# joezie/Personalized-PageRank-Algorithms-on-Neo4j

Hardware: AMD Instinct MI355X
Metric: single-source PPR queries/sec (FORA, alpha=0.15, eps=0.5) (higher is better)
Workload: dtype f64

## Files before the change

### personalized-pagerank-algorithms-on-neo4j_amd/csrc/engine.hpp

```cpp
#pragma once

#include <atomic>
#include <cstdlib>
#include <vector>

#include "common.hpp"

namespace pprhip {

constexpr int kMaxBatch = 8;

struct DevCounters {
  unsigned long long hist[16];
  unsigned long long packed[2];
  double dead[2];
  unsigned long long dead_pops;
  unsigned long long walk_steps;
  unsigned long long walks_total;
  unsigned long long sources_total;
  unsigned long long walk_loads;
  unsigned long long walk_lanes;
  double sum_out;
  unsigned long long mc_plan[3];
  double plan_sum[3];
// ... 164 lines not shown
    if (!last_timed) return;
    last_timed = false;
    hipEvent_t b = next();
    if (b) (void)hipEventRecord(b, stream);
  }
  void add_bytes(int cls, uint64_t bytes) { acc_bytes[cls] += bytes; }
  void reset() {
    used = 0;
    depth = 0;
    last_timed = false;
    recs.clear();
    for (int c = 0; c < 8; ++c) {
      acc_ms[c] = 0.0;
      acc_bytes[c] = 0;
      acc_cnt[c] = 0;
    }
  }
  void resolve(double tot[8], uint64_t bytes[8], uint32_t cnt[8]) {
    fold();
    for (int c = 0; c < 8; ++c) {
      tot[c] += acc_ms[c];
      bytes[c] += acc_bytes[c];
      cnt[c] += acc_cnt[c];
    }
  }
  void destroy() {
    for (hipEvent_t e : ev) (void)hipEventDestroy(e);
    ev.clear();
    reset();
  }
};

struct BatchSync;

constexpr int kBatch = 16;
struct CView {
  double* p;
  uint32_t stride, off;
  __host__ __device__ double& at(uint32_t v) const { return p[(size_t)v * stride + off]; }
};

struct SlotArgs {
  double* res;
  double* reserve;
  uint8_t* flags;
  uint32_t* armed;
  DevCounters* ctr;
  double alpha, rmax, min_rmax;
  int32_t src;
  int32_t active;
  int32_t mode;
  int32_t dead_slot, out_slot;
  int32_t gs_state;
  const double* seed_w;
  const int32_t* seed_id;
  const double* seed_e;
  unsigned int* seed_done;
  uint32_t seed_n_live, seed_n_all;
};

constexpr uint32_t kMailWords = 4112;
struct HostMail {
  unsigned long long seq;
  unsigned long long pad[7];
  unsigned long long words[kMailWords];
};

struct ClearList {
  void* p[6];
  unsigned long long bytes[6];
  int n;
};

struct WalkPlanRec {
  unsigned long long woff;
  double inc;
  unsigned long long ext;
  int32_t node, orig;
};

}

namespace pprhip {
namespace detail {
struct FetchPipe;
}

struct GraphData {
  int device = 0;
  int n_cus = 256;
  uint32_t n = 0;
  uint64_t m = 0;
  uint32_t *out_rp = nullptr, *in_rp = nullptr;
  unsigned long long* out_ext = nullptr;
  int32_t *out_ci = nullptr, *in_ci = nullptr;
  uint4* walk_rec = nullptr;
  std::vector<uint32_t> h_out_rp, h_in_rp;
  bool relabeled = false;
  int32_t *new2old = nullptr, *old2new = nullptr;
  std::vector<int32_t> h_new2old, h_old2new;
  uint8_t* start_flags = nullptr;
  uint32_t* chunk_starts = nullptr;
  uint32_t n_chunks = 0;
  int32_t* nz_rows = nullptr;
  uint32_t n_nz = 0;
  std::vector<int32_t> h_nz_rows;
// ... 240 lines not shown
```

### personalized-pagerank-algorithms-on-neo4j_amd/csrc/fora.cpp

```cpp
#include <algorithm>
#include <atomic>
#include <chrono>
#include <cmath>
#include <condition_variable>
#include <cstdio>
#include <cstring>
#include <functional>
#include <memory>
#include <mutex>
#include <new>
#include <thread>

#include "engine_internal.hpp"

using namespace pprhip;
using namespace pprhip::detail;

namespace pprhip {

struct TopkSchedule {
  double eps = 0, min_delta = 0, m = 0, lg = 0, min_rmax = 0;
  TopkSchedule() = default;
  TopkSchedule(double eps_half, const pprhip_fora_conf_t* conf)
      : eps(eps_half), min_delta(conf->min_delta), m((double)conf->m), lg(std::log(2.0 / conf->pfail)),
// ... 646 lines not shown
  PPRHIP_TRY(check_conf(conf, "pprhip_fora_topk", true));
  PPRHIP_TRY(check_graph(g, "pprhip_fora_topk"));
  PPRHIP_TRY(check_node(g, src, "pprhip_fora_topk"));
  if (!fora_topk_args_ok(conf, eps, cap, ids_out, vals_out, "pprhip_fora_topk")) return PPRHIP_ERR_INVALID;
  ForaRun r;
  PPRHIP_TRY(topk_begin(r, g, g->gr->h_old2new[src], eps, conf, seed, ids_out, vals_out, cap));
  return fora_topk_drive(r, n_out, reserve_out, stats);
}

int pprhip_fora_topk_seeds(pprhip_graph_t* g, const int32_t* seeds, const double* weights, int n_seeds, double eps,
                           const pprhip_fora_conf_t* conf, uint64_t seed, int32_t* ids_out, double* vals_out, int cap,
                           int* n_out, double* reserve_out, pprhip_stats_t* stats) {
  static const char* fn = "pprhip_fora_topk_seeds";
  PPRHIP_TRY(check_positive(eps, fn, "eps"));
  PPRHIP_TRY(check_conf(conf, fn, true));
  PPRHIP_TRY(check_graph(g, fn));
  if (!fora_topk_args_ok(conf, eps, cap, ids_out, vals_out, fn)) return PPRHIP_ERR_INVALID;
  SeedTable plan;
  PPRHIP_TRY(seed_plan(g, seeds, weights, n_seeds, conf->alpha, fn, plan));
  ForaRun r;
  PPRHIP_TRY(topk_begin_seeds(r, g, plan, eps, conf, seed, ids_out, vals_out, cap));
  const int rc = fora_topk_drive(r, n_out, reserve_out, stats);
  g->topk_active = false;
  return rc;
}

namespace {

struct SweepTicket {
  bool active[kBatch] = {false};
  int ws[kBatch] = {0};
  int n_active = 0;
  bool backward = false;
  uint64_t rows = 0;
  unsigned long long seq = 0;
};

int launch_sweep(pprhip_graph* P, ForaRun* runs, const bool* active, int n_active, SweepTicket* T, const int* ws = nullptr) {
  BatchState* bs = P->batch;
  const GraphData* D = P->gr;
  T->n_active = n_active;
  int n_seeded = 0;
  for (int s = 0; s < kBatch; ++s) {
    T->ws[s] = (ws && active[s]) ? ws[s] : s;
    pprhip_graph* S = bs->slots[T->ws[s]];
    SlotArgs& sa = bs->h_slot_args[s];
    T->active[s] = active[s];
    sa.res = S->residue;
    sa.reserve = S->reserve;
    sa.flags = S->flags;
    sa.armed = S->armed;
    sa.ctr = S->ctr;
    sa.active = active[s] ? 1 : 0;
    const SeedTable* sd = (active[s] && S->seed_on) ? S->seeds : nullptr;
    sa.seed_w = sd ? sd->w_node : nullptr;
    sa.seed_id = sd ? sd->id : nullptr;
    sa.seed_e = sd ? sd->w : nullptr;
    sa.seed_done = sd ? sd->done : nullptr;
    sa.seed_n_live = sd ? sd->n_live : 0u;
    sa.seed_n_all = sd ? sd->n_live + sd->n_dead : 0u;
    n_seeded += sd ? 1 : 0;
    if (!active[s]) continue;
    const ForaRun& r = runs[T->ws[s]];
    sa.alpha = r.a.alpha;
    sa.rmax = r.a.rmax;
    sa.min_rmax = r.a.min_rmax;
    sa.src = r.a.src;
    sa.mode = r.a.mode;
    sa.dead_slot = r.L.dslot;
    sa.out_slot = r.L.pslot ^ 1;
    sa.gs_state = r.L.gs_state;
    if (S->stream != P->stream && !S->c8_via_parent) {
      PPRHIP_CHECK_HIP(hipEventRecord(S->ev[3], S->stream));
      PPRHIP_CHECK_HIP(hipStreamWaitEvent(P->stream, S->ev[3], 0));
    }
  }
  bool backward = false;
  for (int s = 0; s < kBatch; ++s)
    if (active[s] && runs[T->ws[s]].a.mode == kBackward) backward = true;
  T->backward = backward;
  const uint64_t rows = backward ? (uint64_t)D->n_nz_o + D->n_z_o : (uint64_t)D->n_nz + D->n_zin;
  T->rows = rows;
  const uint64_t sweep_bytes =
      4ull * D->m + (uint64_t)n_active * (8ull * D->m + 36ull * rows + 4ull) + (uint64_t)n_seeded * 8ull * rows;
  if ((int)backward != bs->acc8_dir) {
    PPRHIP_CHECK_HIP(hipMemsetAsync(bs->acc8, 0, sizeof(double) * ((size_t)D->n + 1) * kBatch, P->stream));
    bs->acc8_dir = (int)backward;
  }
  int n_gs = 1;
  const GsBlock* gs_blocks = backward ? nullptr : gs_blocks_of(bs->slots[0], &n_gs);
#ifdef PPRHIP_TEST_HOOKS
  {
    static const bool on = hook_env("PPRHIP_COUNT_LIVE") != nullptr;
    static unsigned long long* d_cnt = nullptr;
    static unsigned long long sweeps = 0;
    if (on && !backward) {
      if (!d_cnt) {
        PPRHIP_CHECK_HIP(hipMalloc((void**)&d_cnt, 16));
        PPRHIP_CHECK_HIP(hipMemset(d_cnt, 0, 16));
      }
      PPRHIP_TRY(launch_count_live_lines(P, d_cnt));
      if (++sweeps % 200 == 0) {
        unsigned long long h[2];
        PPRHIP_CHECK_HIP(hipMemcpy(h, d_cnt, 16, hipMemcpyDeviceToHost));
        fprintf(stderr, "[pprhip live lines] %llu sweeps: gathers of live lines %.3f of m, live lines %.3f of the sources, busy columns now %d\n",
                sweeps, (double)h[0] / (double)sweeps / (double)D->m, (double)h[1] / (double)sweeps / (double)D->n_src_live, n_active);
      }
    }
  }
#endif
  P->ktimer.begin(PPRHIP_KERNEL_DENSE_PULL_BATCH, sweep_bytes);
  PPRHIP_TRY(launch_dense_level_b8(P, backward, gs_blocks, n_gs));
  P->ktimer.end();
  bs->c8cur ^= 1;
  return fetch_begin(P, bs->sweep_out, sizeof(unsigned long long) * kBatch, &T->seq);
}

bool sweep_arrived(const pprhip_graph* P, const SweepTicket& T) {
  return T.seq != 0 && P->mail && __atomic_load_n(&P->mail->seq, __ATOMIC_ACQUIRE) == T.seq;
}

int collect_sweep(pprhip_graph* P, ForaRun* runs, const SweepTicket& T) {
  PPRHIP_TRY(fetch_end(P, T.seq, P->batch->sweep_out, P->batch->h_sweep_out, sizeof(unsigned long long) * kBatch));
  for (int s = 0; s < kBatch; ++s)
    if (T.active[s]) {
      ForaRun& r = runs[T.ws[s]];
      const unsigned long long pk = P->batch->h_sweep_out[s];
      finish_dense(r.L, r.st, 8ull * P->gr->m + 36ull * T.rows + 4ull + 4ull * P->gr->m / (uint64_t)T.n_active,
                   batch_sweep_min_bytes(P, T.backward, T.n_active) / (uint64_t)T.n_active, (uint32_t)(pk >> kPackShift),
                   pk & kPackMask);
    }
  return PPRHIP_OK;
}

int run_sweep(pprhip_graph* P, ForaRun* runs, const bool* active, int n_active) {
  SweepTicket T;
  PPRHIP_TRY(launch_sweep(P, runs, active, n_active, &T));
// ... 1327 lines not shown
```

### personalized-pagerank-algorithms-on-neo4j_amd/csrc/kernels_push.hip

```cpp
#include <algorithm>
#include <cstdlib>

#include "device_utils.hpp"
#include "engine.hpp"

namespace pprhip {

constexpr int kPushTile = 2048;
constexpr int kStageCap = 512;
constexpr int kCombSlots = 2048;
constexpr int kCombProbes = 4;
constexpr int kCombMinEdges = 262144;

__device__ __forceinline__ bool level_runs(unsigned long long pk, int level, unsigned long long dense_thresh) {
  if (level == 0) return true;
  const unsigned long long nf = pk >> kPackShift, ef = pk & kPackMask;
  if (nf == 0) return false;
  return (nf + ef) < dense_thresh;
}

__device__ __forceinline__ int dense_state(const int* state_in, int state0) { return state_in ? *state_in : state0; }

template <int MODE>
__device__ __forceinline__ void sparse_prepare_body(const int32_t* __restrict__ F, const uint32_t* __restrict__ out_rp,
                                                    double* __restrict__ res, double* __restrict__ reserve,
                                                    double* __restrict__ cF, CView c_dense, DevCounters* ctr, int level,
                                                    int dead_slot, unsigned long long pk0, unsigned long long pk,
                                                    const PushArgs& a, uint32_t bid, uint32_t nblk) {
  __shared__ double s_red[4];
  __shared__ unsigned long long s_red2[4];
  if (level == 0 && pk0 != ~0ull && bid == 0 && threadIdx.x == 0) {
    for (int i = 1; i <= kMaxBatch; ++i) ctr->hist[i] = 0ull;
    ctr->hist[kMaxBatch + 2] = 0ull;
  }
  const uint32_t nf = (uint32_t)(pk >> kPackShift);
  double dead = 0.0;
  unsigned long long ndead = 0;
  for (uint32_t i = bid * blockDim.x + threadIdx.x; i < nf; i += nblk * blockDim.x) {
    const int32_t v = F[i];
    const double rc = res[v];
    res[v] = 0.0;
    reserve[v] = reserve[v] + rc * a.alpha;
    double c;
    if (MODE == kBackward) {
      c = (1.0 - a.alpha) * rc;
    } else {
      const uint32_t d = out_rp[v + 1] - out_rp[v];
      if (d == 0) {
        c = 0.0;
        dead += rc * (1.0 - a.alpha);
        ndead++;
      } else {
        c = ((1.0 - a.alpha) * rc) / (double)d;
// ... 810 lines not shown
    if (MODE == kBackward) {
      if (acc > 0.0) {
        const double old = res[u];
        const double nw = old + acc / (double)d;
        if (!(old > a.rmax) && nw > a.rmax) {
          reserve[u] = reserve[u] + nw * a.alpha;
          if (old != 0.0) res[u] = 0.0;
          cn = (1.0 - a.alpha) * nw;
          pack = (1ull << kPackShift) | (unsigned long long)(in_rp[u + 1] - in_rp[u]);
        } else {
          res[u] = nw;
        }
      }
    } else if (acc > 0.0) {
      const double old = res[u];
      const double nw = old + acc;
      bool crossing = (MODE == kPower) ? true : (!active_fwd(old, d, a.rmax) && active_fwd(nw, d, a.rmax));
      if (MODE == kFwdTopk) {
        if (a.rmax < a.min_rmax && active_fwd(old, d, a.rmax)) crossing = take_armed(armed, u);
        if (active_fwd(nw, d, a.min_rmax)) flags[u] = 1;
      }
      if (crossing) {
        reserve[u] = reserve[u] + nw * a.alpha;
        if (old != 0.0) res[u] = 0.0;
        if (d == 0) {
          dead_next = nw * (1.0 - a.alpha);
          ndead = 1;
        } else {
          cn = ((1.0 - a.alpha) * nw) / (double)d;
        }
        pack = (1ull << kPackShift) | (unsigned long long)d;
      } else {
        res[u] = nw;
      }
    }
    c_next[u] = cn;
    if (!last_block) {
      if (state == kGsEntry) c_cur[u] = c_cur[u] + cn;
      else if (state == kGsInPlace) c_cur[u] = cn;
      else if (state == kGsFlush) c_cur[u] = 0.0;
    }
  }
  const double ds = block_sum_f64(dead_next, s_red);
  const unsigned long long ps = block_sum_u64(pack, s_red2);
  const unsigned long long nd = block_sum_u64(ndead, s_red2);
  if (tid == 0) {
    blk_pack[blockIdx.x] = ps;
    blk_dead[blockIdx.x] = ds;
    blk_ndead[blockIdx.x] = (uint32_t)nd;
  }
}

constexpr int kApplyRows = 64;
constexpr int kApplyGroups = 2;
constexpr int kApplyThreads = 512;
constexpr int kSlotsPerWave = kBatch / (kApplyThreads / 64);

__global__ __launch_bounds__(kApplyThreads) void k_dense_apply_batch(const int32_t* __restrict__ nz_rows, uint32_t n_nz,
                                                            const int32_t* __restrict__ zin_rows, uint32_t n_zin,
                                                            double* __restrict__ acc8,
                                                            const uint32_t* __restrict__ out_rp,
                                                            const uint32_t* __restrict__ in_rp_bwd,
                                                            double* __restrict__ c8_cur, double* __restrict__ c8_next,
                                                            uint32_t tile_lo, uint32_t tile_hi, uint32_t gs_mask,
                                                            uint32_t entry_mask,
                                                            const SlotArgs* __restrict__ slots,
                                                            const unsigned long long* __restrict__ cross_bits,
                                                            unsigned long long* __restrict__ prep_bits,
                                                            unsigned long long* __restrict__ blk_pack8,
                                                            double* __restrict__ blk_dead8,
                                                            uint32_t* __restrict__ blk_ndead8, uint32_t part_base,
                                                            uint32_t part_stride) {
  __shared__ double tile[kApplyGroups][kApplyRows][kBatch + 1];
  __shared__ double tile_p[kApplyGroups][kApplyRows][kBatch + 1];
  __shared__ int32_t s_u[kApplyGroups][kApplyRows];
  __shared__ uint32_t s_d[kApplyGroups][kApplyRows];
  __shared__ uint32_t s_din[kApplyGroups][kApplyRows];
  const int tid = threadIdx.x, lane = tid & 63;
  const int w = __builtin_amdgcn_readfirstlane(tid >> 6);
  const uint32_t n_rows = n_nz + n_zin;
  const uint32_t n_tiles = (n_rows + kApplyRows - 1) / kApplyRows;
  SlotArgs a[kSlotsPerWave];
#pragma unroll
  for (int i = 0; i < kSlotsPerWave; ++i) a[i] = slots[w * kSlotsPerWave + i];
  double dead_next[kSlotsPerWave];
  unsigned long long pack[kSlotsPerWave];
  uint32_t ndead[kSlotsPerWave];
#pragma unroll
  for (int i = 0; i < kSlotsPerWave; ++i) {
    dead_next[i] = 0.0;
    pack[i] = 0;
    ndead[i] = 0;
  }
  for (uint32_t tl0 = tile_lo + blockIdx.x * kApplyGroups; tl0 < tile_hi; tl0 += gridDim.x * kApplyGroups) {
#pragma unroll
    for (int g = 0; g < kApplyGroups; ++g) {
      const uint32_t tl = tl0 + g;
      const bool in = tl < tile_hi;
      const uint32_t row0 = tl * kApplyRows;
      const unsigned long long cw = in ? cross_bits[tl] : 0ull;
#pragma unroll
      for (int i = 0; i < kApplyRows * kBatch / kApplyThreads; ++i) {
        const uint32_t idx = (uint32_t)i * (uint32_t)kApplyThreads + tid;
        const uint32_t r = idx / kBatch, s = idx % kBatch;
        const uint32_t j = row0 + r;
        double v = 0.0;
        if (in && j < n_nz) {
          const size_t t = (size_t)j * kBatch + s;
          v = __builtin_nontemporal_load(&acc8[t]);
          if (v != 0.0 && ((cw >> r) & 1ull)) acc8[t] = 0.0;
        }
// ... 88 lines not shown
          }
          if (crossing) {
            a[i].reserve[u[g]] = rsvv[g][i] + nw * a[i].alpha;
            if (oldv[g][i] != 0.0) a[i].res[u[g]] = 0.0;
            if (d[g] == 0) {
              dead_next[i] += nw * (1.0 - a[i].alpha);
              ndead[i]++;
            } else {
              cn = ((1.0 - a[i].alpha) * nw) / (double)d[g];
            }
            pack[i] += (1ull << kPackShift) | (unsigned long long)d[g];
          } else {
            a[i].res[u[g]] = nw;
          }
        }
        tile[g][lane][s] = cn;
        if (gs_mask >> s & 1u) {
          const int gst = a[i].gs_state;
          tile_p[g][lane][s] = gst == kGsEntry ? tile_p[g][lane][s] + cn : (gst == kGsInPlace ? cn : 0.0);
        }
        const unsigned long long bits = __ballot(cn > 0.0);
        if (lane == 0 && a[i].active && tl0 + g < tile_hi) prep_bits[(size_t)s * n_tiles + tl0 + g] = bits;
      }
    }
    __syncthreads();
#pragma unroll
    for (int g = 0; g < kApplyGroups; ++g) {
#pragma unroll
      for (int i = 0; i < kApplyRows * kBatch / kApplyThreads; ++i) {
        const uint32_t idx = (uint32_t)i * (uint32_t)kApplyThreads + tid;
        const uint32_t r = idx / kBatch, s = idx % kBatch;
        const int32_t ur = s_u[g][r];
        if (ur >= 0) {
          c8_next[(size_t)ur * kBatch + s] = tile[g][r][s];
          if (gs_mask >> s & 1u) c8_cur[(size_t)ur * kBatch + s] = tile_p[g][r][s];
        }
      }
    }
    __syncthreads();
  }
#pragma unroll
  for (int i = 0; i < kSlotsPerWave; ++i) {
    const double ds = wave_sum_f64(dead_next[i]);
    const unsigned long long ps = wave_sum_u64(pack[i]);
    const unsigned long long nd = wave_sum_u64((unsigned long long)ndead[i]);
    if (lane == 0) {
      const size_t o = (size_t)(w * kSlotsPerWave + i) * part_stride + part_base + blockIdx.x;
      blk_pack8[o] = ps;
      blk_dead8[o] = ds;
      blk_ndead8[o] = (uint32_t)nd;
    }
  }
}

__global__ __launch_bounds__(1024) void k_dense_reduce_batch(const unsigned long long* __restrict__ blk_pack8,
                                                           const double* __restrict__ blk_dead8,
                                                           const uint32_t* __restrict__ blk_ndead8, uint32_t n_blocks,
                                                           uint32_t part_stride,
                                                           const SlotArgs* __restrict__ slots,
                                                           unsigned long long* __restrict__ sweep_out) {
  __shared__ double s_red[16];
  __shared__ unsigned long long s_red2[16];
  const SlotArgs a = slots[blockIdx.x];
  if (!a.active) return;
  unsigned long long pack = 0, ndead = 0;
  double dead = 0.0;
  for (uint32_t i = threadIdx.x; i < n_blocks; i += blockDim.x) {
    pack += blk_pack8[(size_t)blockIdx.x * part_stride + i];
    dead += blk_dead8[(size_t)blockIdx.x * part_stride + i];
    ndead += blk_ndead8[(size_t)blockIdx.x * part_stride + i];
  }
  const unsigned long long ps = block_sum_u64(pack, s_red2);
  const unsigned long long nd = block_sum_u64(ndead, s_red2);
  const double ds = block_sum_f64(dead, s_red);
  if (threadIdx.x == 0) {
    a.ctr->packed[a.out_slot] = ps;
    sweep_out[blockIdx.x] = ps;
    if (nd) {
      a.ctr->dead[a.dead_slot ^ 1] = a.ctr->dead[a.dead_slot ^ 1] + ds;
      a.ctr->dead_pops += nd;
    }
  }
}

__global__ __launch_bounds__(1024) void k_dense_reduce(const unsigned long long* __restrict__ blk_pack,
                                                        const double* __restrict__ blk_dead,
                                                        const uint32_t* __restrict__ blk_ndead, uint32_t n_blocks,
                                                        DevCounters* ctr, int out_slot, int dead_slot_next,
                                                        const int* state_in, int state0, unsigned long long* hist_out,
                                                        int* state_out, unsigned long long dense_thresh,
                                                        unsigned long long gs_thresh, uint32_t* queues) {
  __shared__ double s_red[16];
  __shared__ unsigned long long s_red2[16];
  if (queues && threadIdx.x < kPanelQueues) queues[threadIdx.x] = 0u;
  const int state = dense_state(state_in, state0);
  if (state == kGsNone) {
    if (threadIdx.x == 0 && state_out) *state_out = kGsNone;
    return;
  }
  unsigned long long pack = 0, ndead = 0;
  double dead = 0.0;
  for (uint32_t i = threadIdx.x; i < n_blocks; i += blockDim.x) {
    pack += blk_pack[i];
    if (blk_dead) {
      dead += blk_dead[i];
      ndead += blk_ndead[i];
    }
  }
  const unsigned long long ps = block_sum_u64(pack, s_red2);
  const unsigned long long nd = block_sum_u64(ndead, s_red2);
  const double ds = block_sum_f64(dead, s_red);
  if (threadIdx.x == 0) {
    ctr->packed[out_slot] = ps;
    if (hist_out) *hist_out = ps;
    if (state_out) *state_out = gs_next_state(state, ps >> kPackShift, ps & kPackMask, dense_thresh, gs_thresh);
    if (nd) {
      ctr->dead[dead_slot_next] = ctr->dead[dead_slot_next] + ds;
      ctr->dead_pops += nd;
    }
  }
}

template <int KIND>
__device__ __forceinline__ bool seed_pred(uint32_t v, const double* __restrict__ res, uint32_t d,
                                          const uint8_t* __restrict__ flags, const PushArgs& a) {
  if (KIND == 1 && !flags[v]) return false;
  return active_fwd(res[v], d, a.rmax);
}

__device__ __forceinline__ void unpark(uint32_t v, const double* __restrict__ res, uint32_t d,
                                       uint8_t* __restrict__ flags, const PushArgs& a) {
  if (!flags[v]) return;
  const double r = res[v];
  if (active_fwd(r, d, a.rmax) || !active_fwd(r, d, a.min_rmax)) flags[v] = 0;
}

template <int KIND>
// ... 537 lines not shown
  const uint32_t c_hi = (uint32_t)((B.e_hi + kChunkEdges - 1) / kChunkEdges);
  const uint32_t want = (c_hi - c_lo + 15) / 16;
  const unsigned long long* flags64 = reinterpret_cast<const unsigned long long*>(start_flags);
  if (n_hot) {
    const uint32_t grid = std::min<uint32_t>(want, (uint32_t)g->gr->n_cus);
    k_dense_edges_b<true, G><<<dim3(grid), dim3(1024), sizeof(double) * n_hot * G, g->stream>>>(
        ci, flags64, chunk_starts, c_hi, (unsigned long long)g->gr->m, cB, accB, n_hot, c_lo, B.e_lo, B.e_hi, g->gr->n);
  } else {
    const uint32_t grid = std::min<uint32_t>(want, (uint32_t)g->gr->n_cus * 2u);
    k_dense_edges_b<false, G><<<dim3(grid), dim3(1024), 0, g->stream>>>(
        ci, flags64, chunk_starts, c_hi, (unsigned long long)g->gr->m, cB, accB, 0u, c_lo, B.e_lo, B.e_hi, g->gr->n);
  }
  PPRHIP_CHECK_HIP(hipGetLastError());
  return PPRHIP_OK;
}

#ifdef PPRHIP_TEST_HOOKS
__global__ __launch_bounds__(256) void k_count_live_lines(const double* __restrict__ c8, const uint32_t* __restrict__ out_rp,
                                                          uint32_t n, unsigned long long* out) {
  __shared__ unsigned long long s_red[4];
  const uint32_t v = blockIdx.x * 256u + threadIdx.x;
  unsigned long long d = 0, c = 0;
  if (v < n) {
    bool live = false;
    for (int s = 0; s < kBatch; ++s) live |= c8[(size_t)v * kBatch + s] != 0.0;
    if (live) {
      d = out_rp[v + 1] - out_rp[v];
      c = 1;
    }
  }
  const unsigned long long ds = block_sum_u64(d, s_red), cs = block_sum_u64(c, s_red);
  if (threadIdx.x == 0 && (ds | cs)) {
    atomicAdd(&out[0], ds);
    atomicAdd(&out[1], cs);
  }
}
int launch_count_live_lines(pprhip_graph* P, unsigned long long* d_out) {
  const BatchState* bs = P->batch;
  k_count_live_lines<<<dim3((P->gr->n + 255) / 256), dim3(256), 0, P->stream>>>(bs->c8[bs->c8cur], P->gr->out_rp, P->gr->n,
                                                                              d_out);
  PPRHIP_CHECK_HIP(hipGetLastError());
  return PPRHIP_OK;
}
#endif

#ifdef PPRHIP_TEST_HOOKS
int launch_sweep_edges_only(pprhip_graph* P, const GsBlock& B) {
  const GraphData* D = P->gr;
  const BatchState* bs = P->batch;
  return launch_dense_edges_bG<kBatch>(P, D->in_ci, D->start_flags, D->chunk_starts, bs->c8[bs->c8cur], bs->acc8, B);
}
#endif

int launch_dense_level_b8(pprhip_graph* P, bool backward, const GsBlock* gs_blocks, int n_gs_blocks) {
  const GraphData* D = P->gr;
  const BatchState* bs = P->batch;
  PPRHIP_CHECK_HIP(hipMemcpyAsync(bs->d_slot_args, bs->h_slot_args, sizeof(SlotArgs) * kBatch, hipMemcpyHostToDevice,
                                  P->stream));
  const int32_t* ci = backward ? D->out_ci : D->in_ci;
  const uint8_t* flags = backward ? D->start_flags_o : D->start_flags;
  const uint32_t* cstarts = backward ? D->chunk_starts_o : D->chunk_starts;
  const int32_t* nz = backward ? D->nz_rows_o : D->nz_rows;
  const int32_t* zr = backward ? D->z_rows_o : D->zin_rows;
  const uint32_t n_nz = backward ? D->n_nz_o : D->n_nz, n_z = backward ? D->n_z_o : D->n_zin;
  const unsigned long long* cross = backward ? D->cross_bits_o : D->cross_bits;
  uint32_t gs_mask = 0, entry_mask = 0;
  for (int s = 0; s < kBatch; ++s)
    if (bs->h_slot_args[s].active) {
      const int st = bs->h_slot_args[s].gs_state;
      if (st == kGsEntry || st == kGsInPlace || st == kGsFlush) gs_mask |= 1u << s;
      if (st == kGsEntry) entry_mask |= 1u << s;
    }
  const uint32_t n_rows = n_nz + n_z;
  const uint32_t n_tiles = (n_rows + kApplyRows - 1) / kApplyRows;
  const GsBlock whole{0u, n_nz, 0ull, (unsigned long long)D->m};
  const bool cut = gs_mask && gs_blocks && n_gs_blocks > 1 && !backward;
  const GsBlock* blocks = cut ? gs_blocks : &whole;
  const int nb = cut ? n_gs_blocks : 1;
  uint32_t part_base = 0;
  for (int b = 0; b < nb; ++b) {
    const GsBlock& B = blocks[b];
    PPRHIP_TRY(launch_dense_edges_bG<kBatch>(P, ci, flags, cstarts, bs->c8[bs->c8cur], bs->acc8, B));
    const uint32_t t_lo = B.j_lo / kApplyRows;
    const uint32_t t_hi = (b == nb - 1) ? n_tiles : B.j_hi / kApplyRows;
    if (t_hi <= t_lo) continue;
    const uint32_t quota = kApplyBlocks8 / (uint32_t)nb;
    const uint32_t grid = std::max(1u, std::min((t_hi - t_lo + kApplyGroups - 1) / kApplyGroups, quota));
    k_dense_apply_batch<<<dim3(grid), dim3(kApplyThreads), 0, P->stream>>>(
          nz, n_nz, zr, n_z, bs->acc8, D->out_rp, backward ? D->in_rp : nullptr, bs->c8[bs->c8cur], bs->c8[bs->c8cur ^ 1], t_lo,
          t_hi, b == nb - 1 ? 0u : gs_mask, b == nb - 1 ? 0u : entry_mask, bs->d_slot_args, cross, bs->prep_bits,
          bs->blk_pack8, bs->blk_dead8, bs->blk_ndead8, part_base, kApplyBlocks8);
    PPRHIP_CHECK_HIP(hipGetLastError());
    part_base += grid;
  }
  uint32_t seed_dead_max = 0;
  bool seeded = false;
  for (int s = 0; s < kBatch; ++s) {
    const SlotArgs& sa = bs->h_slot_args[s];
    if (sa.active && sa.seed_w && !backward) {
      seeded = true;
      seed_dead_max = std::max(seed_dead_max, sa.seed_n_all - sa.seed_n_live);
    }
  }
  if (seeded) {
    k_seed_land_dense_batch<<<dim3(grid_for(seed_dead_max, 256, 1024), kBatch), dim3(256), 0, P->stream>>>(
        bs->d_slot_args);
    PPRHIP_CHECK_HIP(hipGetLastError());
  }
  k_dense_reduce_batch<<<dim3(kBatch), dim3(1024), 0, P->stream>>>(bs->blk_pack8, bs->blk_dead8, bs->blk_ndead8, part_base,
                                                                   kApplyBlocks8, bs->d_slot_args, bs->sweep_out);
  PPRHIP_CHECK_HIP(hipGetLastError());
  return PPRHIP_OK;
}

int launch_compact_prepared(pprhip_graph* g, int cbuf, int out_fbuf, unsigned long long* d_counter, bool backward) {
  const uint32_t grid = grid_for(g->gr->n, 1024, 1024);
  if (g->parent) {
    const GraphData* D = g->gr;
    const uint32_t n_rows = backward ? D->n_nz_o + D->n_z_o : D->n_nz + D->n_zin;
    const uint32_t n_tiles = (n_rows + kApplyRows - 1) / kApplyRows;
    k_compact_bits<<<dim3(grid), dim3(256), 0, g->stream>>>(
        n_rows, backward ? D->n_nz_o : D->n_nz, g->parent->batch->prep_bits + (size_t)g->slot_index * n_tiles,
        backward ? D->nz_rows_o : D->nz_rows, backward ? D->z_rows_o : D->zin_rows, cview(g, cbuf),
        backward ? D->in_rp : D->out_rp, g->F[out_fbuf], g->eoff[out_fbuf], g->cF, d_counter);
  } else {
    k_compact_prepared<<<dim3(grid), dim3(256), 0, g->stream>>>(act_n(g), cview(g, cbuf), false,
                                                                backward ? g->gr->in_rp : g->gr->out_rp, g->F[out_fbuf],
                                                                g->eoff[out_fbuf], g->cF, d_counter);
  }
  PPRHIP_CHECK_HIP(hipGetLastError());
  return PPRHIP_OK;
}

static int reduce_partials(pprhip_graph* g, uint32_t n_blocks, int out_slot, int dead_slot, bool with_dead) {
  k_dense_reduce<<<dim3(1), dim3(1024), 0, g->stream>>>(g->blk_pack, with_dead ? g->blk_dead : nullptr, g->blk_ndead,
                                                        n_blocks, g->ctr, out_slot, dead_slot, nullptr, kGsJacobi, nullptr,
                                                        nullptr, 0ull, ~0ull, nullptr);
  PPRHIP_CHECK_HIP(hipGetLastError());
  return PPRHIP_OK;
}

// ... 127 lines not shown
```

Measured before the change: 346.7.

## Skip residue loads for rows known zero via previous-sweep prep bits

Adds a new dense apply kernel that uses per-tile prep bits written by the previous sweep to skip loading residue (and often reserve) for rows known to hold zero residue, when the slot is in whole-forward mode with a prior dense run. The kernel also double-buffers the shared tile so the write-out of the previous tile overlaps the next tile's work, and it records ballot bits of nonzero outputs for the next sweep. The old kernel is kept behind an environment switch, and the bandwidth estimate is reduced accordingly. The risk is correctness if the prep bits go stale, plus extra shared memory and register pressure.

```diff
diff --git a/personalized-pagerank-algorithms-on-neo4j_amd/csrc/engine.hpp b/personalized-pagerank-algorithms-on-neo4j_amd/csrc/engine.hpp
--- a/personalized-pagerank-algorithms-on-neo4j_amd/csrc/engine.hpp
+++ b/personalized-pagerank-algorithms-on-neo4j_amd/csrc/engine.hpp
@@ -240,6 +240,7 @@
   int32_t mode;
   int32_t dead_slot, out_slot;
   int32_t gs_state;
+  int32_t prep_ok;
   const double* seed_w;
   const int32_t* seed_id;
   const double* seed_e;
diff --git a/personalized-pagerank-algorithms-on-neo4j_amd/csrc/fora.cpp b/personalized-pagerank-algorithms-on-neo4j_amd/csrc/fora.cpp
--- a/personalized-pagerank-algorithms-on-neo4j_amd/csrc/fora.cpp
+++ b/personalized-pagerank-algorithms-on-neo4j_amd/csrc/fora.cpp
@@ -722,6 +722,7 @@
     sa.armed = S->armed;
     sa.ctr = S->ctr;
     sa.active = active[s] ? 1 : 0;
+    sa.prep_ok = 0;
     const SeedTable* sd = (active[s] && S->seed_on) ? S->seeds : nullptr;
     sa.seed_w = sd ? sd->w_node : nullptr;
     sa.seed_id = sd ? sd->id : nullptr;
@@ -740,6 +741,7 @@
     sa.dead_slot = r.L.dslot;
     sa.out_slot = r.L.pslot ^ 1;
     sa.gs_state = r.L.gs_state;
+    sa.prep_ok = (r.a.mode == kFwdWhole && r.L.dense_run > 0) ? 1 : 0;
     if (S->stream != P->stream && !S->c8_via_parent) {
       PPRHIP_CHECK_HIP(hipEventRecord(S->ev[3], S->stream));
       PPRHIP_CHECK_HIP(hipStreamWaitEvent(P->stream, S->ev[3], 0));
@@ -751,8 +753,10 @@
   T->backward = backward;
   const uint64_t rows = backward ? (uint64_t)D->n_nz_o + D->n_z_o : (uint64_t)D->n_nz + D->n_zin;
   T->rows = rows;
-  const uint64_t sweep_bytes =
-      4ull * D->m + (uint64_t)n_active * (8ull * D->m + 36ull * rows + 4ull) + (uint64_t)n_seeded * 8ull * rows;
+  int n_prep = 0;
+  for (int s = 0; s < kBatch; ++s) n_prep += active[s] && bs->h_slot_args[s].prep_ok ? 1 : 0;
+  const uint64_t sweep_bytes = 4ull * D->m + (uint64_t)n_active * (8ull * D->m + 36ull * rows + 4ull) +
+                               (uint64_t)n_seeded * 8ull * rows - (uint64_t)n_prep * 8ull * rows;
   if ((int)backward != bs->acc8_dir) {
     PPRHIP_CHECK_HIP(hipMemsetAsync(bs->acc8, 0, sizeof(double) * ((size_t)D->n + 1) * kBatch, P->stream));
     bs->acc8_dir = (int)backward;
diff --git a/personalized-pagerank-algorithms-on-neo4j_amd/csrc/kernels_push.hip b/personalized-pagerank-algorithms-on-neo4j_amd/csrc/kernels_push.hip
--- a/personalized-pagerank-algorithms-on-neo4j_amd/csrc/kernels_push.hip
+++ b/personalized-pagerank-algorithms-on-neo4j_amd/csrc/kernels_push.hip
@@ -1,4 +1,5 @@
 #include <algorithm>
+#include <atomic>
 #include <cstdlib>
 
 #include "device_utils.hpp"
@@ -919,7 +920,7 @@
 constexpr int kApplyThreads = 512;
 constexpr int kSlotsPerWave = kBatch / (kApplyThreads / 64);
 
-__global__ __launch_bounds__(kApplyThreads) void k_dense_apply_batch(const int32_t* __restrict__ nz_rows, uint32_t n_nz,
+__global__ __launch_bounds__(kApplyThreads) void k_dense_apply_batch_prev(const int32_t* __restrict__ nz_rows, uint32_t n_nz,
                                                             const int32_t* __restrict__ zin_rows, uint32_t n_zin,
                                                             double* __restrict__ acc8,
                                                             const uint32_t* __restrict__ out_rp,
@@ -1145,6 +1146,242 @@
   }
 }
 
+__global__ __launch_bounds__(kApplyThreads) void k_dense_apply_batch(const int32_t* __restrict__ nz_rows, uint32_t n_nz,
+                                                            const int32_t* __restrict__ zin_rows, uint32_t n_zin,
+                                                            double* __restrict__ acc8,
+                                                            const uint32_t* __restrict__ out_rp,
+                                                            const uint32_t* __restrict__ in_rp_bwd,
+                                                            double* __restrict__ c8_cur, double* __restrict__ c8_next,
+                                                            uint32_t tile_lo, uint32_t tile_hi, uint32_t gs_mask,
+                                                            uint32_t entry_mask,
+                                                            const SlotArgs* __restrict__ slots,
+                                                            const unsigned long long* __restrict__ cross_bits,
+                                                            unsigned long long* __restrict__ prep_bits,
+                                                            unsigned long long* __restrict__ blk_pack8,
+                                                            double* __restrict__ blk_dead8,
+                                                            uint32_t* __restrict__ blk_ndead8, uint32_t part_base,
+                                                            uint32_t part_stride) {
+  constexpr int kPer = kApplyRows * kBatch / kApplyThreads;
+  __shared__ double tile[2][kApplyGroups][kApplyRows][kBatch + 1];
+  __shared__ double tile_p[kApplyGroups][kApplyRows][kBatch + 1];
+  __shared__ int32_t s_u[2][kApplyGroups][kApplyRows];
+  __shared__ uint32_t s_d[2][kApplyGroups][kApplyRows];
+  __shared__ uint32_t s_din[2][kApplyGroups][kApplyRows];
+  const int tid = threadIdx.x, lane = tid & 63;
+  const int w = __builtin_amdgcn_readfirstlane(tid >> 6);
+  const uint32_t n_rows = n_nz + n_zin;
+  const uint32_t n_tiles = (n_rows + kApplyRows - 1) / kApplyRows;
+  SlotArgs a[kSlotsPerWave];
+#pragma unroll
+  for (int i = 0; i < kSlotsPerWave; ++i) a[i] = slots[w * kSlotsPerWave + i];
+  double dead_next[kSlotsPerWave];
+  unsigned long long pack[kSlotsPerWave];
+  uint32_t ndead[kSlotsPerWave];
+#pragma unroll
+  for (int i = 0; i < kSlotsPerWave; ++i) {
+    dead_next[i] = 0.0;
+    pack[i] = 0;
+    ndead[i] = 0;
+  }
+  double nv[kApplyGroups][kPer];
+  unsigned long long ncw[kApplyGroups];
+  int32_t nu = -1;
+  uint32_t nd = 0, ndin = 0;
+  const uint32_t step = gridDim.x * kApplyGroups;
+  auto load_sums = [&](uint32_t t0) {
+#pragma unroll
+    for (int g = 0; g < kApplyGroups; ++g) {
+      const uint32_t tl = t0 + g;
+      const bool in = tl < tile_hi;
+      ncw[g] = in ? cross_bits[tl] : 0ull;
+#pragma unroll
+      for (int i = 0; i < kPer; ++i) {
+        const uint32_t idx = (uint32_t)i * (uint32_t)kApplyThreads + tid;
+        const uint32_t j = tl * kApplyRows + idx / kBatch;
+        nv[g][i] = (in && j < n_nz) ? __builtin_nontemporal_load(&acc8[(size_t)j * kBatch + idx % kBatch]) : 0.0;
+      }
+    }
+    if (tid < kApplyRows * kApplyGroups) {
+      const uint32_t tl = t0 + tid / kApplyRows;
+      const uint32_t j = tl * kApplyRows + tid % kApplyRows;
+      nu = tl >= tile_hi ? -1 : (j < n_nz ? nz_rows[j] : (j < n_rows ? zin_rows[j - n_nz] : -1));
+    }
+  };
+  auto load_degrees = [&]() {
+    if (tid < kApplyRows * kApplyGroups) {
+      nd = nu >= 0 ? out_rp[nu + 1] - out_rp[nu] : 0u;
+      ndin = (nu >= 0 && in_rp_bwd) ? in_rp_bwd[nu + 1] - in_rp_bwd[nu] : 0u;
+    }
+  };
+  auto write_out = [&](int b) {
+#pragma unroll
+    for (int g = 0; g < kApplyGroups; ++g) {
+#pragma unroll
+      for (int i = 0; i < kPer; ++i) {
+        const uint32_t idx = (uint32_t)i * (uint32_t)kApplyThreads + tid;
+        const uint32_t r = idx / kBatch, s = idx % kBatch;
+        const int32_t ur = s_u[b][g][r];
+        if (ur >= 0) {
+          c8_next[(size_t)ur * kBatch + s] = tile[b][g][r][s];
+          if (gs_mask >> s & 1u) c8_cur[(size_t)ur * kBatch + s] = tile_p[g][r][s];
+        }
+      }
+    }
+  };
+  uint32_t tl0 = tile_lo + blockIdx.x * kApplyGroups;
+  if (tl0 < tile_hi) {
+    load_sums(tl0);
+    load_degrees();
+  }
+  int buf = 0;
+  bool pending = false;
+  for (; tl0 < tile_hi; tl0 += step) {
+#pragma unroll
+    for (int g = 0; g < kApplyGroups; ++g) {
+      const uint32_t tl = tl0 + g;
+#pragma unroll
+      for (int i = 0; i < kPer; ++i) {
+        const uint32_t idx = (uint32_t)i * (uint32_t)kApplyThreads + tid;
+        const uint32_t r = idx / kBatch, s = idx % kBatch;
+        const uint32_t j = tl * kApplyRows + r;
+        const double v = nv[g][i];
+        if (v != 0.0 && ((ncw[g] >> r) & 1ull)) acc8[(size_t)j * kBatch + s] = 0.0;
+        tile[buf][g][r][s] = v;
+      }
+    }
+    if (tid < kApplyRows * kApplyGroups) {
+      const uint32_t g = tid / kApplyRows, r = tid % kApplyRows;
+      s_u[buf][g][r] = nu;
+      s_d[buf][g][r] = nd;
+      s_din[buf][g][r] = ndin;
+    }
+    if (pending) write_out(buf ^ 1);
+    __syncthreads();
+    if (entry_mask) {
+#pragma unroll
+      for (int g = 0; g < kApplyGroups; ++g) {
+#pragma unroll
+        for (int i = 0; i < kPer; ++i) {
+          const uint32_t idx = (uint32_t)i * (uint32_t)kApplyThreads + tid;
+          const uint32_t r = idx / kBatch, s = idx % kBatch;
+          const int32_t ur = s_u[buf][g][r];
+          tile_p[g][r][s] = (ur >= 0 && (entry_mask >> s & 1u)) ? c8_cur[(size_t)ur * kBatch + s] : 0.0;
+        }
+      }
+      __syncthreads();
+    }
+    load_sums(tl0 + step);
+    int32_t u[kApplyGroups];
+    uint32_t d[kApplyGroups], din[kApplyGroups];
+    double accv[kApplyGroups][kSlotsPerWave], oldv[kApplyGroups][kSlotsPerWave], rsvv[kApplyGroups][kSlotsPerWave];
+    bool live[kApplyGroups][kSlotsPerWave];
+#pragma unroll
+    for (int g = 0; g < kApplyGroups; ++g) {
+      u[g] = s_u[buf][g][lane];
+      d[g] = s_d[buf][g][lane];
+      din[g] = s_din[buf][g][lane];
+#pragma unroll
+      for (int i = 0; i < kSlotsPerWave; ++i) {
+        double acc = tile[buf][g][lane][w * kSlotsPerWave + i];
+        const bool on = a[i].active && u[g] >= 0;
+        if (on && a[i].mode != kBackward && u[g] == a[i].src) {
+          const double dd = a[i].ctr->dead[a[i].dead_slot];
+          if (dd > 0.0) {
+            acc += dd;
+            a[i].ctr->dead[a[i].dead_slot] = 0.0;
+          }
+        } else if (a[i].seed_w && a[i].mode != kBackward) {
+          const double x = a[i].ctr->dead[a[i].dead_slot];
+          if (x > 0.0 && on) {
+            const double sw = a[i].seed_w[u[g]];
+            if (sw != 0.0) acc += x * sw;
+          }
+        }
+        accv[g][i] = acc;
+        live[g][i] = on && acc > 0.0;
+      }
+    }
+#pragma unroll
+    for (int g = 0; g < kApplyGroups; ++g) {
+#pragma unroll
+      for (int i = 0; i < kSlotsPerWave; ++i) {
+        const int s = w * kSlotsPerWave + i;
+        const unsigned long long pb =
+            (a[i].prep_ok && tl0 + g < tile_hi) ? prep_bits[(size_t)s * n_tiles + tl0 + g] : 0ull;
+        const bool zero = (pb >> lane) & 1ull;
+        const bool cross0 = zero && !active_fwd(0.0, d[g], a[i].rmax) && active_fwd(accv[g][i], d[g], a[i].rmax);
+        oldv[g][i] = live[g][i] && !zero ? a[i].res[u[g]] : 0.0;
+        rsvv[g][i] = live[g][i] && (!zero || cross0) ? a[i].reserve[u[g]] : 0.0;
+      }
+    }
+    load_degrees();
+#pragma unroll
+    for (int g = 0; g < kApplyGroups; ++g) {
+#pragma unroll
+      for (int i = 0; i < kSlotsPerWave; ++i) {
+        const int s = w * kSlotsPerWave + i;
+        double cn = 0.0;
+        if (live[g][i] && a[i].mode == kBackward) {
+          const double old = oldv[g][i];
+          const double nw = old + accv[g][i] / (double)d[g];
+          if (!(old > a[i].rmax) && nw > a[i].rmax) {
+            a[i].reserve[u[g]] = rsvv[g][i] + nw * a[i].alpha;
+            if (oldv[g][i] != 0.0) a[i].res[u[g]] = 0.0;
+            cn = (1.0 - a[i].alpha) * nw;
+            pack[i] += (1ull << kPackShift) | (unsigned long long)din[g];
+          } else {
+            a[i].res[u[g]] = nw;
+          }
+        } else if (live[g][i]) {
+          const double old = oldv[g][i];
+          const double nw = old + accv[g][i];
+          bool crossing = !active_fwd(old, d[g], a[i].rmax) && active_fwd(nw, d[g], a[i].rmax);
+          if (a[i].mode == kFwdTopk) {
+            if (a[i].rmax < a[i].min_rmax && active_fwd(old, d[g], a[i].rmax)) crossing = take_armed(a[i].armed, u[g]);
+            if (active_fwd(nw, d[g], a[i].min_rmax)) a[i].flags[u[g]] = 1;
+          }
+          if (crossing) {
+            a[i].reserve[u[g]] = rsvv[g][i] + nw * a[i].alpha;
+            if (oldv[g][i] != 0.0) a[i].res[u[g]] = 0.0;
+            if (d[g] == 0) {
+              dead_next[i] += nw * (1.0 - a[i].alpha);
+              ndead[i]++;
+            } else {
+              cn = ((1.0 - a[i].alpha) * nw) / (double)d[g];
+            }
+            pack[i] += (1ull << kPackShift) | (unsigned long long)d[g];
+          } else {
+            a[i].res[u[g]] = nw;
+          }
+        }
+        tile[buf][g][lane][s] = cn;
+        if (gs_mask >> s & 1u) {
+          const int gst = a[i].gs_state;
+          tile_p[g][lane][s] = gst == kGsEntry ? tile_p[g][lane][s] + cn : (gst == kGsInPlace ? cn : 0.0);
+        }
+        const unsigned long long bits = __ballot(cn > 0.0);
+        if (lane == 0 && a[i].active && tl0 + g < tile_hi) prep_bits[(size_t)s * n_tiles + tl0 + g] = bits;
+      }
+    }
+    __syncthreads();
+    pending = true;
+    buf ^= 1;
+  }
+  if (pending) write_out(buf ^ 1);
+#pragma unroll
+  for (int i = 0; i < kSlotsPerWave; ++i) {
+    const double ds = wave_sum_f64(dead_next[i]);
+    const unsigned long long ps = wave_sum_u64(pack[i]);
+    const unsigned long long nq = wave_sum_u64((unsigned long long)ndead[i]);
+    if (lane == 0) {
+      const size_t o = (size_t)(w * kSlotsPerWave + i) * part_stride + part_base + blockIdx.x;
+      blk_pack8[o] = ps;
+      blk_dead8[o] = ds;
+      blk_ndead8[o] = (uint32_t)nq;
+    }
+  }
+}
+
 __global__ __launch_bounds__(1024) void k_dense_reduce(const unsigned long long* __restrict__ blk_pack,
                                                         const double* __restrict__ blk_dead,
                                                         const uint32_t* __restrict__ blk_ndead, uint32_t n_blocks,
@@ -1788,11 +2025,26 @@
 }
 #endif
 
+static bool apply_prev() { return hook_env("PPRHIP_APPLY_PREV") != nullptr; }
+
+#ifdef PPRHIP_TEST_HOOKS
+static bool sweep_fail_now() {
+  static std::atomic<long> n{0};
+  const char* e = hook_env("PPRHIP_SWEEP_FAIL_AT");
+  if (!e) {
+    n = 0;
+    return false;
+  }
+  return n++ == atol(e);
+}
+#endif
+
 int launch_dense_level_b8(pprhip_graph* P, bool backward, const GsBlock* gs_blocks, int n_gs_blocks) {
   const GraphData* D = P->gr;
   const BatchState* bs = P->batch;
   PPRHIP_CHECK_HIP(hipMemcpyAsync(bs->d_slot_args, bs->h_slot_args, sizeof(SlotArgs) * kBatch, hipMemcpyHostToDevice,
                                   P->stream));
+  const bool prev = apply_prev();
   const int32_t* ci = backward ? D->out_ci : D->in_ci;
   const uint8_t* flags = backward ? D->start_flags_o : D->start_flags;
   const uint32_t* cstarts = backward ? D->chunk_starts_o : D->chunk_starts;
@@ -1817,12 +2069,24 @@
   for (int b = 0; b < nb; ++b) {
     const GsBlock& B = blocks[b];
     PPRHIP_TRY(launch_dense_edges_bG<kBatch>(P, ci, flags, cstarts, bs->c8[bs->c8cur], bs->acc8, B));
+#ifdef PPRHIP_TEST_HOOKS
+    if (b == 0 && sweep_fail_now()) {
+      set_error("batched sweep: injected failure between the edge and apply launches (PPRHIP_SWEEP_FAIL_AT)");
+      return PPRHIP_ERR_STATE;
+    }
+#endif
     const uint32_t t_lo = B.j_lo / kApplyRows;
     const uint32_t t_hi = (b == nb - 1) ? n_tiles : B.j_hi / kApplyRows;
     if (t_hi <= t_lo) continue;
     const uint32_t quota = kApplyBlocks8 / (uint32_t)nb;
     const uint32_t grid = std::max(1u, std::min((t_hi - t_lo + kApplyGroups - 1) / kApplyGroups, quota));
-    k_dense_apply_batch<<<dim3(grid), dim3(kApplyThreads), 0, P->stream>>>(
+    if (prev)
+      k_dense_apply_batch_prev<<<dim3(grid), dim3(kApplyThreads), 0, P->stream>>>(
+          nz, n_nz, zr, n_z, bs->acc8, D->out_rp, backward ? D->in_rp : nullptr, bs->c8[bs->c8cur], bs->c8[bs->c8cur ^ 1], t_lo,
+          t_hi, b == nb - 1 ? 0u : gs_mask, b == nb - 1 ? 0u : entry_mask, bs->d_slot_args, cross, bs->prep_bits,
+          bs->blk_pack8, bs->blk_dead8, bs->blk_ndead8, part_base, kApplyBlocks8);
+    else
+      k_dense_apply_batch<<<dim3(grid), dim3(kApplyThreads), 0, P->stream>>>(
           nz, n_nz, zr, n_z, bs->acc8, D->out_rp, backward ? D->in_rp : nullptr, bs->c8[bs->c8cur], bs->c8[bs->c8cur ^ 1], t_lo,
           t_hi, b == nb - 1 ? 0u : gs_mask, b == nb - 1 ? 0u : entry_mask, bs->d_slot_args, cross, bs->prep_bits,
           bs->blk_pack8, bs->blk_dead8, bs->blk_ndead8, part_base, kApplyBlocks8);
```

After: 348.3, median of 6. Within noise of the previous version (+0.5%).

## Rewrite dense batch apply as persistent wave-per-tile kernel with prefetch

Applied to the files above, without the earlier changes.

Replaces the 512-thread block-synchronised dense apply kernel with a 4-wave kernel in which each wave owns a 64-row tile, syncs only within the wavefront, and software-prefetches the next tile's accumulator values and row ids while processing the current one. The grid is capped at two workgroups per CU so waves loop persistently over tiles. Per-slot reductions move into registers and are combined across waves once at the end. The old kernel is kept behind a test-hook environment switch. The aim is to cut block-wide barriers and expose memory latency overlap, at the cost of lower occupancy and added register pressure from the prefetch buffers.

```diff
diff --git a/personalized-pagerank-algorithms-on-neo4j_amd/csrc/kernels_push.hip b/personalized-pagerank-algorithms-on-neo4j_amd/csrc/kernels_push.hip
--- a/personalized-pagerank-algorithms-on-neo4j_amd/csrc/kernels_push.hip
+++ b/personalized-pagerank-algorithms-on-neo4j_amd/csrc/kernels_push.hip
@@ -915,11 +915,13 @@
 }
 
 constexpr int kApplyRows = 64;
+
+#ifdef PPRHIP_TEST_HOOKS
 constexpr int kApplyGroups = 2;
 constexpr int kApplyThreads = 512;
 constexpr int kSlotsPerWave = kBatch / (kApplyThreads / 64);
 
-__global__ __launch_bounds__(kApplyThreads) void k_dense_apply_batch(const int32_t* __restrict__ nz_rows, uint32_t n_nz,
+__global__ __launch_bounds__(kApplyThreads) void k_dense_apply_batch_trips(const int32_t* __restrict__ nz_rows, uint32_t n_nz,
                                                             const int32_t* __restrict__ zin_rows, uint32_t n_zin,
                                                             double* __restrict__ acc8,
                                                             const uint32_t* __restrict__ out_rp,
@@ -1114,6 +1116,247 @@
     }
   }
 }
+#endif
+
+constexpr int kApplyWaves = 4;
+constexpr int kApplyWgPerCu = 2;
+constexpr int kLineRows = 64 / kBatch;
+
+__device__ __forceinline__ void wave_lds_sync() {
+  __builtin_amdgcn_fence(__ATOMIC_RELEASE, "wavefront");
+  __builtin_amdgcn_wave_barrier();
+  __builtin_amdgcn_fence(__ATOMIC_ACQUIRE, "wavefront");
+}
+
+template <typename T>
+__device__ __forceinline__ T* opaque(T* p) {
+  uint32_t z = 0;
+  asm volatile("" : "+s"(z));
+  return p + z;
+}
+
+__global__ __launch_bounds__(64 * kApplyWaves) void k_dense_apply_batch(const int32_t* __restrict__ nz_rows, uint32_t n_nz,
+                                                            const int32_t* __restrict__ zin_rows, uint32_t n_zin,
+                                                            double* __restrict__ acc8,
+                                                            const uint32_t* __restrict__ out_rp,
+                                                            const uint32_t* __restrict__ in_rp_bwd,
+                                                            double* __restrict__ c8_cur, double* __restrict__ c8_next,
+                                                            uint32_t tile_lo, uint32_t tile_hi, uint32_t gs_mask,
+                                                            uint32_t entry_mask,
+                                                            const SlotArgs* __restrict__ slots,
+                                                            const unsigned long long* __restrict__ cross_bits,
+                                                            unsigned long long* __restrict__ prep_bits,
+                                                            unsigned long long* __restrict__ blk_pack8,
+                                                            double* __restrict__ blk_dead8,
+                                                            uint32_t* __restrict__ blk_ndead8, uint32_t part_base,
+                                                            uint32_t part_stride) {
+  __shared__ double tile[kApplyWaves][kApplyRows][kBatch + 1];
+  __shared__ int32_t s_u[kApplyWaves][kApplyRows];
+  __shared__ uint32_t s_d[kApplyWaves][kApplyRows];
+  __shared__ uint32_t s_din[kApplyWaves][kApplyRows];
+  __shared__ unsigned long long s_pack[kApplyWaves][kBatch];
+  __shared__ double s_dead[kApplyWaves][kBatch];
+  __shared__ uint32_t s_nd[kApplyWaves][kBatch];
+  const int lane = threadIdx.x & 63;
+  const int w = __builtin_amdgcn_readfirstlane(threadIdx.x >> 6);
+  const uint32_t ls = lane % kBatch, lr = lane / kBatch;
+  double(*T)[kBatch + 1] = tile[w];
+  const uint32_t n_rows = n_nz + n_zin;
+  const uint32_t n_tiles = (n_rows + kApplyRows - 1) / kApplyRows;
+  uint32_t act_m = 0, bwd_m = 0, inpl_m = 0;
+#pragma unroll
+  for (int s = 0; s < kBatch; ++s) {
+    act_m |= slots[s].active ? 1u << s : 0u;
+    bwd_m |= slots[s].mode == kBackward ? 1u << s : 0u;
+    inpl_m |= slots[s].gs_state == kGsInPlace ? 1u << s : 0u;
+  }
+  const bool l_bwd = bwd_m >> ls & 1u, l_gs = gs_mask >> ls & 1u, l_entry = entry_mask >> ls & 1u,
+             l_inpl = inpl_m >> ls & 1u;
+  unsigned long long pack_l = 0;
+  double dead_l = 0.0;
+  uint32_t nd_l = 0;
+
+  const uint32_t stride = gridDim.x * kApplyWaves;
+  uint32_t tl = tile_lo + blockIdx.x * kApplyWaves + w;
+  double nx[kApplyRows / kLineRows];
+  int32_t nu = -1;
+  auto fetch = [&](uint32_t t) {
+    const uint32_t row0 = t * kApplyRows;
+#pragma unroll
+    for (int k = 0; k < kApplyRows / kLineRows; ++k) {
+      const uint32_t j = row0 + (uint32_t)k * kLineRows + lr;
+      const double x = __builtin_nontemporal_load(&acc8[(size_t)(j < n_nz ? j : 0u) * kBatch + ls]);
+      nx[k] = j < n_nz ? x : 0.0;
+    }
+    const uint32_t j = row0 + lane;
+    const uint32_t jq = j < n_rows ? j : n_rows - 1;
+    const int32_t x = jq < n_nz ? nz_rows[jq] : zin_rows[jq - n_nz];
+    nu = j < n_rows ? x : -1;
+  };
+  if (tl < tile_hi) fetch(tl);
+  for (; tl < tile_hi; tl += stride) {
+    const SlotArgs* sl = opaque(slots);
+    const uint32_t row0 = tl * kApplyRows;
+    const int32_t u = nu;
+    {
+      const unsigned long long cw = cross_bits[tl];
+#pragma unroll
+      for (int k = 0; k < kApplyRows / kLineRows; ++k) {
+        const uint32_t r = (uint32_t)k * kLineRows + lr;
+        T[r][ls] = nx[k];
+        if (nx[k] != 0.0 && ((cw >> r) & 1ull)) acc8[(size_t)(row0 + r) * kBatch + ls] = 0.0;
+      }
+    }
+    wave_lds_sync();
+    uint32_t live_m = 0;
+#pragma unroll
+    for (int s = 0; s < kBatch; ++s) {
+      const SlotArgs& A = sl[s];
+      const bool on = (act_m >> s & 1u) && u >= 0;
+      double acc = T[lane][s];
+      if (on && A.mode != kBackward && u == A.src) {
+        const double dd = A.ctr->dead[A.dead_slot];
+        if (dd > 0.0) {
+          acc += dd;
+          A.ctr->dead[A.dead_slot] = 0.0;
+          T[lane][s] = acc;
+        }
+      } else if ((act_m >> s & 1u) && A.seed_w && A.mode != kBackward) {
+        const double x = A.ctr->dead[A.dead_slot];
+        if (x > 0.0 && on) {
+          const double sw = A.seed_w[u];
+          if (sw != 0.0) {
+            acc += x * sw;
+            T[lane][s] = acc;
+          }
+        }
+      }
+      live_m |= (on && acc > 0.0) ? 1u << s : 0u;
+    }
+    const uint32_t uc = u >= 0 ? (uint32_t)u : 0u;
+    const uint32_t* dp = in_rp_bwd ? in_rp_bwd : out_rp;
+    const uint32_t d0 = out_rp[uc], d1 = out_rp[uc + 1], e0 = dp[uc], e1 = dp[uc + 1];
+    double oldv[kBatch], rsvv[kBatch];
+#pragma unroll
+    for (int s = 0; s < kBatch; ++s) {
+      const bool act = act_m >> s & 1u;
+      const double* rp = act ? sl[s].res : acc8;
+      const double* qp = act ? sl[s].reserve : acc8;
+      const uint32_t ui = (live_m >> s & 1u) ? uc : 0u;
+      oldv[s] = rp[ui];
+      rsvv[s] = qp[ui];
+    }
+    if (tl + stride < tile_hi) fetch(tl + stride);
+    const uint32_t d = u >= 0 ? d1 - d0 : 0u, din = u >= 0 ? e1 - e0 : 0u;
+    s_u[w][lane] = u;
+    s_d[w][lane] = d;
+    s_din[w][lane] = din;
+    const unsigned long long zb = __ballot(d == 0);
+    const SlotArgs* sm = opaque(slots);
+    unsigned long long bcl = 0, pbl = 0;
+#pragma unroll
+    for (int s = 0; s < kBatch; ++s) {
+      const SlotArgs& A = sm[s];
+      const bool live = live_m >> s & 1u;
+      const double acc = T[lane][s];
+      double cn = 0.0, dn = 0.0;
+      bool crossing = false;
+      if (live && A.mode == kBackward) {
+        const double old = oldv[s];
+        const double nw = old + acc / (double)d;
+        if (!(old > A.rmax) && nw > A.rmax) {
+          A.reserve[u] = rsvv[s] + nw * A.alpha;
+          if (old != 0.0) A.res[u] = 0.0;
+          cn = (1.0 - A.alpha) * nw;
+          crossing = true;
+        } else {
+          A.res[u] = nw;
+        }
+      } else if (live) {
+        const double old = oldv[s];
+        const double nw = old + acc;
+        crossing = !active_fwd(old, d, A.rmax) && active_fwd(nw, d, A.rmax);
+        if (A.mode == kFwdTopk) {
+          if (A.rmax < A.min_rmax && active_fwd(old, d, A.rmax)) crossing = take_armed(A.armed, u);
+          if (active_fwd(nw, d, A.min_rmax)) A.flags[u] = 1;
+        }
+        if (crossing) {
+          A.reserve[u] = rsvv[s] + nw * A.alpha;
+          if (old != 0.0) A.res[u] = 0.0;
+          if (d == 0) dn = nw * (1.0 - A.alpha);
+          else cn = ((1.0 - A.alpha) * nw) / (double)d;
+        } else {
+          A.res[u] = nw;
+        }
+      }
+      T[lane][s] = (d == 0 && !(bwd_m >> s & 1u)) ? dn : cn;
+      const unsigned long long bc = __ballot(crossing), pb = __ballot(cn > 0.0);
+      if (ls == (uint32_t)s) {
+        bcl = bc;
+        pbl = pb;
+        pack_l += (unsigned long long)__popcll(bc) << kPackShift;
+        if (!(bwd_m >> s & 1u)) nd_l += (uint32_t)__popcll(bc & zb);
+      }
+    }
+    if (lane < kBatch && (act_m >> lane & 1u)) prep_bits[(size_t)lane * n_tiles + tl] = pbl;
+    wave_lds_sync();
+    double pc[kApplyRows / kLineRows];
+    if (entry_mask) {
+#pragma unroll
+      for (int k = 0; k < kApplyRows / kLineRows; ++k) {
+        const int32_t ur = s_u[w][k * kLineRows + lr];
+        pc[k] = c8_cur[(size_t)(ur >= 0 ? ur : 0) * kBatch + ls];
+      }
+    }
+    uint32_t degsum = 0;
+    double deadsum = 0.0;
+#pragma unroll
+    for (int k = 0; k < kApplyRows / kLineRows; ++k) {
+      const uint32_t r = (uint32_t)k * kLineRows + lr;
+      const double t = T[r][ls];
+      const int32_t ur = s_u[w][r];
+      const uint32_t dr = s_d[w][r];
+      const bool dz = dr == 0 && !l_bwd;
+      const double cn = dz ? 0.0 : t;
+      if (dz) deadsum += t;
+      if ((bcl >> r) & 1ull) degsum += l_bwd ? s_din[w][r] : dr;
+      if (ur >= 0) {
+        const size_t o = (size_t)ur * kBatch + ls;
+        c8_next[o] = cn;
+        if (l_gs) c8_cur[o] = l_entry ? pc[k] + cn : (l_inpl ? cn : 0.0);
+      }
+    }
+    degsum += __shfl_xor(degsum, 16);
+    degsum += __shfl_xor(degsum, 32);
+    deadsum += __shfl_xor(deadsum, 16);
+    deadsum += __shfl_xor(deadsum, 32);
+    pack_l += degsum;
+    dead_l += deadsum;
+    wave_lds_sync();
+  }
+  if (lane < kBatch) {
+    s_pack[w][lane] = pack_l;
+    s_dead[w][lane] = dead_l;
+    s_nd[w][lane] = nd_l;
+  }
+  __syncthreads();
+  if (threadIdx.x < kBatch) {
+    const int s = threadIdx.x;
+    unsigned long long ps = 0;
+    double ds = 0.0;
+    uint32_t nd = 0;
+#pragma unroll
+    for (int v = 0; v < kApplyWaves; ++v) {
+      ps += s_pack[v][s];
+      ds += s_dead[v][s];
+      nd += s_nd[v][s];
+    }
+    const size_t o = (size_t)s * part_stride + part_base + blockIdx.x;
+    blk_pack8[o] = ps;
+    blk_dead8[o] = ds;
+    blk_ndead8[o] = nd;
+  }
+}
 
 __global__ __launch_bounds__(1024) void k_dense_reduce_batch(const unsigned long long* __restrict__ blk_pack8,
                                                            const double* __restrict__ blk_dead8,
@@ -1788,6 +2031,13 @@
 }
 #endif
 
+#ifdef PPRHIP_TEST_HOOKS
+static bool apply_trips() {
+  const char* e = hook_env("PPRHIP_APPLY_BATCH");
+  return e && e[0] == '0';
+}
+#endif
+
 int launch_dense_level_b8(pprhip_graph* P, bool backward, const GsBlock* gs_blocks, int n_gs_blocks) {
   const GraphData* D = P->gr;
   const BatchState* bs = P->batch;
@@ -1821,8 +2071,22 @@
     const uint32_t t_hi = (b == nb - 1) ? n_tiles : B.j_hi / kApplyRows;
     if (t_hi <= t_lo) continue;
     const uint32_t quota = kApplyBlocks8 / (uint32_t)nb;
-    const uint32_t grid = std::max(1u, std::min((t_hi - t_lo + kApplyGroups - 1) / kApplyGroups, quota));
-    k_dense_apply_batch<<<dim3(grid), dim3(kApplyThreads), 0, P->stream>>>(
+    uint32_t grid;
+#ifdef PPRHIP_TEST_HOOKS
+    if (apply_trips()) {
+      grid = std::max(1u, std::min((t_hi - t_lo + kApplyGroups - 1) / kApplyGroups, quota));
+      k_dense_apply_batch_trips<<<dim3(grid), dim3(kApplyThreads), 0, P->stream>>>(
+          nz, n_nz, zr, n_z, bs->acc8, D->out_rp, backward ? D->in_rp : nullptr, bs->c8[bs->c8cur], bs->c8[bs->c8cur ^ 1], t_lo,
+          t_hi, b == nb - 1 ? 0u : gs_mask, b == nb - 1 ? 0u : entry_mask, bs->d_slot_args, cross, bs->prep_bits,
+          bs->blk_pack8, bs->blk_dead8, bs->blk_ndead8, part_base, kApplyBlocks8);
+      PPRHIP_CHECK_HIP(hipGetLastError());
+      part_base += grid;
+      continue;
+    }
+#endif
+    grid = std::max(1u, std::min({(t_hi - t_lo + kApplyWaves - 1) / kApplyWaves,
+                                  (uint32_t)D->n_cus * (uint32_t)kApplyWgPerCu, quota}));
+    k_dense_apply_batch<<<dim3(grid), dim3(64 * kApplyWaves), 0, P->stream>>>(
           nz, n_nz, zr, n_z, bs->acc8, D->out_rp, backward ? D->in_rp : nullptr, bs->c8[bs->c8cur], bs->c8[bs->c8cur ^ 1], t_lo,
           t_hi, b == nb - 1 ? 0u : gs_mask, b == nb - 1 ? 0u : entry_mask, bs->d_slot_args, cross, bs->prep_bits,
           bs->blk_pack8, bs->blk_dead8, bs->blk_ndead8, part_base, kApplyBlocks8);
```

Result: slower. 354.0 before, 347.0 after (median of 2 runs) (-2.0%).
